# pnnl/FragNet

Measured on AMD Instinct MI355X. Metric: molecules/sec fwd+bwd (full training step), ESOL-shape batch=512 per GPU, higher is better.
Workload: dtype f32; 1 GPU; ESOL finetune batch=512 fp32 (BASELINE configs[1]): FragNetFineTune 4 layers x 4 heads, emb 128, FTHead3 128/1024/1024/512, drop 0.1; synthetic ESOL-shape molecules (synth.py); per_gpu_batch=512, global_batch=512, parallelism=dp1, overlap=off, graph_replays=736, eager_fallbacks=0, step=plan+zero_grad+fwd+mse+bwd+adam, atoms=13334, bond_graph_edges=200112

## Files before the change

### fragnet_amd/csrc/encoder.hip

```cpp
#include <hip/hip_runtime.h>
#include <algorithm>
#include <mutex>
#include <stdint.h>

#include "fn_internal.h"

namespace {
using fni::fail;
using fni::launch_status;
using fni::tune;
using fni::prof_event;
using fni::GatFwdArgs;
using fni::prep_gat_fwd;
using fni::launch_gat_fwd;
using fni::launch_gat_fwd_pair;
using fni::launch_gat_fwd_lin;
using fni::launch_gat_fwd_pair_lin;
using fni::GatBwdOneArgs;
using fni::CuTask;
using fni::CuTasks;
using fni::prep_gat_bwd_one;
using fni::launch_gat_bwd_one3;
using fni::launch_gat_cu;
using fni::launch_linear128_group;
// ... 7 lines not shown
#include "shared_bodies.inc"

constexpr int kRowDotsBwdBlocks = 512;

struct RowDotsBwdArgs {
    const float *g_s_sorted, *feat, *A;
    int lda, off, J;
    fn_gat_plan pl;
    float* g_feat;
    float* part;
    const float* addend;
    int g_is_orig, nblk;
    const float *cu_out2, *cu_sigma;
    float *cu_c, *cu_u;
    const int32_t* n_real;
};
__device__ __forceinline__ void row_dots_sorted_bwd_range(const RowDotsBwdArgs& T, float (*sR)[FN_D], int64_t e0, int64_t e1, int vb) {
    const float* __restrict__ g_s_sorted = T.g_s_sorted;
    const float* __restrict__ feat = T.feat;
    const float* __restrict__ A = T.A;
    const int lda = T.lda, off = T.off, J = T.J, g_is_orig = T.g_is_orig;
    const fn_gat_plan& pl = T.pl;
    float* g_feat = T.g_feat;
    float* __restrict__ part = T.part;
    const float* addend = T.addend;
    const int lane = threadIdx.x & 31, hw = threadIdx.x >> 5;
    float4 a[8], q[8];
#pragma unroll
    for (int i = 0; i < 8; ++i) {
        a[i] = (i < J) ? ld4(A + i * lda + off + lane * 4) : make_float4(0.f, 0.f, 0.f, 0.f);
// ... 45 lines not shown
                fma4(q[i], gs, v);
            }
        }
        if (addend) { const float4 a0 = ld4(addend + e * FN_D + lane * 4); acc.x += a0.x; acc.y += a0.y; acc.z += a0.z; acc.w += a0.w; }
        st4(g_feat + e * FN_D + lane * 4, acc);
    }
#pragma unroll
    for (int i = 0; i < 8; ++i) {
        if (i < J) {
            st4(&sR[hw][lane * 4], q[i]);
            __syncthreads();
            if (threadIdx.x < FN_D) {
                float v = 0.f;
#pragma unroll
                for (int w = 0; w < kRows; ++w) v += sR[w][threadIdx.x];
                part[(size_t)(i * FN_D + threadIdx.x) * FN_MAX_PART + vb] = v;
            }
            __syncthreads();
        }
    }
}
__device__ __forceinline__ void row_dots_sorted_bwd_body(const RowDotsBwdArgs& T, float (*sR)[FN_D], int vb, int nb) {
    const int64_t m_live = T.n_real && *T.n_real < T.pl.m_real ? (int64_t)*T.n_real : T.pl.m_real;
    const int64_t groups = (T.pl.m_real + kRows - 1) / kRows, per = (groups + nb - 1) / nb;
    const int64_t live_blocks = (m_live + per * kRows - 1) / (per * kRows);
    const int64_t g0 = (int64_t)xcd_block_real(vb, nb, (int)(live_blocks < nb ? live_blocks : nb)) * per, g1 = g0 + per < groups ? g0 + per : groups;
    const int64_t e1 = g1 * kRows < m_live ? g1 * kRows : m_live;
    row_dots_sorted_bwd_range(T, sR, g0 * kRows < e1 ? g0 * kRows : e1, e1, vb);
}
__global__ __launch_bounds__(kBlock) void k_row_dots_sorted_bwd(RowDotsBwdArgs T) {
    __shared__ float sR[kRows][FN_D];
// ... 322 lines not shown
    return o;
}

bool have_mol(const fn_encoder* e) {
    return e->n_mols > 0 && e->mol_atoms.rowptr && e->mol_frags.rowptr && e->mol_atoms.n_seg == e->n_mols && e->mol_frags.n_seg == e->n_mols;
}
bool pad_skip_on(const fn_encoder* e) {
    return tune(FN_TUNE_PAD_SKIP) != 0 && one_pass_on(e) && have_mol(e) && e->mol_contiguous != 0 && e->counts_dev != nullptr && e->variant == 0;
}
bool tail_mol_on(const fn_encoder* e) {
    return tune(FN_TUNE_MOL_TAIL) != 0 && e->mol_contiguous != 0 && have_mol(e) && e->variant == 0 &&
           (e->heads == 2 || e->heads == 4 || e->heads == 8) && e->F > 0 && e->EF > 0 && e->frag.m > 1 && e->n_mols <= FN_MAX_PART &&
           !((uintptr_t)e->ws & 15);
}

struct LevelScratch {
    float *g_h, *dz, *pz, *g_s_dst, *part_a, *part_e, *part_rd, *wg_ws;
    float* cdot;
};
struct BwdLayout {
    float* g_pre[kLevels + 1];
    float* g_frags;
    LevelScratch lv[FN_MAX_LAYERS][kLevels], frag;
    int64_t total;
};

BwdLayout bwd_layout(const fn_encoder* e, float* ws) {
    BwdLayout o{};
    Bump b(ws);
    const int H = e->heads;
// ... 118 lines not shown
    if (et.mode == 0) et.s_sorted = s_sorted;
    return et;
}
inline NodeScalarEpi node_scalars(const LevelView& v) { return NodeScalarEpi{v.att, v.s_dst, v.s_src, v.att_w, 0, v.src_off, v.H}; }
inline LinTask proj_task(const LevelView& v, int k_task = 0) {
    LinTask t{v.W, v.x, v.Wt, v.bias, v.a.h, v.rows, fn_act_epilogue{nullptr, 0.f, 0, 0, 0, nullptr}, node_scalars(v), 0, 0, k_task};
    t.n_real = v.n_real;
    return t;
}

struct ParamWork {
    int n_a = 0, n_e = 0;
    int n_rd = 0;
};
inline fni::AttParamGrads att_param_grads(const LevelView& v, const LevelWeights& g, const LevelScratch& sc, int n_a, int n_e) {
    return fni::AttParamGrads{v.H, sc.part_a, n_a, sc.part_e, n_e, v.et, v.att, v.att_w, v.src_off, g.att, g.embW, g.embb};
}
int edge_term_colsum(ParamGradQueue& rq, const LevelView& v, const LevelWeights& g, const LevelScratch& sc, int n_rd) {
    return rq.colsum(sc.part_rd, n_rd, v.H * FN_D, g.att, v.att_w, v.mid_off);
}
int level_params(ParamGradQueue& rq, const LevelView& v, const LevelWeights& g, const LevelScratch& sc, const ParamWork& o, hipStream_t launch_on) {
    FN_TRY(rq.finalize(att_param_grads(v, g, sc, o.n_a, o.n_e)));
    if (o.n_rd) FN_TRY(edge_term_colsum(rq, v, g, sc, o.n_rd));
    return rq.wgrad(fni::ProjWgrad{sc.g_h, v.x, v.K, v.rows, sc.wg_ws, v.n_real, g.W, g.bias}, launch_on);
}

int launch_gat_bwd_src(const GatBwdSrcArgs& A, int heads, hipStream_t st) {
    if (A.nblk == 0) return 0;
    FN_TRY(with_heads(heads, [&](auto H) { hipLaunchKernelGGL((k_gat_bwd_src<FN_CV(H), kBwdRows>), dim3(A.nblk), dim3(kBwdRows * 32), 0, st, A); }));
    return launch_status("fn_gat_bwd_src_f32");
}

int bwd_src_and_edge_term(const LevelView& v, const LevelScratch& sc, const float* g_out, float* g_h, const float* feat, float* g_feat,
                          bool accumulate, int* n_part_a, int* n_rd, hipStream_t st) {
    const int heads = v.H;
    GatBwdSrcArgs A;
    if (int rc = prep_gat_bwd_src(g_out, v.a.h, sc.pz, sc.g_s_dst, v.att, v.att_w, 0, v.src_off, v.pl, g_h, sc.part_a, n_part_a, heads, &A)) return rc;
    *n_rd = v.pl->m_real > 0 ? row_grid(v.pl->m_real, tune(FN_TUNE_RD_BLOCKS) > 0 ? tune(FN_TUNE_RD_BLOCKS) : kRowDotsBwdBlocks) : 0;
    if (*n_rd == 0) return launch_gat_bwd_src(A, heads, st);
    const RowDotsBwdArgs T{sc.dz, feat, v.att, v.att_w, v.mid_off, heads, *v.pl, g_feat, sc.part_rd, accumulate ? (const float*)g_feat : nullptr, 1, *n_rd};
    if (A.nblk == 0) {
        hipLaunchKernelGGL(k_row_dots_sorted_bwd, dim3(T.nblk), dim3(kBlock), 0, st, T);
        return launch_status("edge-term backward");
    }
    FN_TRY(with_heads(heads, [&](auto H) { hipLaunchKernelGGL((k_gat_bwd_src_rd<FN_CV(H), kBwdRows>), dim3(A.nblk + T.nblk), dim3(kBlock), 0, st, A, T); }));
    return launch_status("source pass + edge-term backward");
}

static int launch_lin_rd(LinTasks& T, const RowDotsBwdArgs& R, hipStream_t st) {
    int blocks = 0, live = 0;
    bool aligned = true;
    for (int i = 0; i < T.n; ++i) {
        if (T.t[i].M <= 0) continue;
        LinTask t = T.t[i];
        if (((uintptr_t)t.X | (uintptr_t)t.Bt | (uintptr_t)t.Y | (uintptr_t)t.bias | (uintptr_t)t.mk.y) & 15) aligned = false;
// ... 52 lines not shown
int launch_tail_bwd(const fn_encoder* e, const EncLayout& lay, const BwdLayout& bw, const EncOutputs& y, const EncOutputs& gy, bool accumulate_fbond,
                    int* n_part, hipStream_t st, bool one_pass_dots = false, bool* rider_done = nullptr) {
    const int H = e->heads, l = e->n_layers - 1;
    const LevelView vf = level_view(e, lay, l, LV_FRAG), va = level_view(e, lay, l, LV_ATOM), vfb = level_view(e, lay, l, LV_FBOND);
    const LevelScratch& sf = bw.frag;
    const float *y_atoms = y.y[LV_ATOM], *y_frags = y.y[LV_FRAG], *g_atoms = gy.y[LV_ATOM], *g_frags = gy.y[LV_FRAG];
    TailBwdArgs T{};
    T.ext = reinterpret_cast<const MolExt*>(lay.mol_ext);  T.n_mols = (int)e->n_mols;  T.counts_dev = e->counts_dev;
    T.g_atoms = g_atoms;  T.g_frags = g_frags;  T.g_pooled = e->g_pooled;  T.y_atoms = y_atoms;  T.y_frags = y_frags;  T.scale = gate_scale(e);
    T.g_pre_atoms = bw.g_pre[LV_ATOM];  T.g_pre_frags = bw.g_pre[LV_FRAG];  T.a2f_index = e->a2f.index;  T.n_atoms = e->N;  T.force_global = tune(FN_TUNE_MOL_TAIL) == 2;
    int n_e = 0, n_a = 0;
    FN_TRY(prep_gat_bwd_dst(bw.g_pre[LV_FRAG], vf.a.h, vf.a.p, &vf.et, vf.pl, 0.2f, nullptr, sf.dz, sf.pz, sf.g_s_dst, nullptr, &n_e, H, &T.D));
    FN_TRY(prep_gat_bwd_src(bw.g_pre[LV_FRAG], vf.a.h, sf.pz, sf.g_s_dst, vf.att, vf.att_w, 0, vf.src_off, vf.pl, bw.g_frags, sf.part_a, &n_a, H, &T.S));
    T.R = RowDotsBwdArgs{sf.dz, vfb.a.raw, vf.att, vf.att_w, vf.mid_off, H, *vf.pl, bw.g_pre[LV_FBOND], sf.part_rd,
                         accumulate_fbond ? (const float*)bw.g_pre[LV_FBOND] : (const float*)nullptr, 1, 0};
    if (one_pass_dots) {
        const LevelScratch &sa = bw.lv[l][LV_ATOM], &sfb = bw.lv[l][LV_FBOND];
        T.cu_out = va.a.raw;  T.cu_out2 = va.a.o2;  T.cu_sigma = va.a.sg;  T.cu_c = sa.cdot;  T.cu_u = sa.g_s_dst;
        if (H == 4) { T.R.cu_out2 = vfb.a.o2;  T.R.cu_sigma = vfb.a.sg;  T.R.cu_c = sfb.cdot;  T.R.cu_u = sfb.g_s_dst; }
    }
    if (((uintptr_t)y_atoms | (uintptr_t)y_frags | (uintptr_t)g_atoms | (uintptr_t)g_frags | (uintptr_t)e->g_pooled) & 15)
        return fail(FN_EINVAL, "fragment tail backward: gradients must be 16-byte aligned");
    AdamRide R{};
    if (rider_done) {
        *rider_done = false;
        if (tune(FN_TUNE_RIDER_AT) == 1 && e->adam_rider) {
            R = make_adam_ride(e->adam_rider, (int)e->n_mols, kBlock, tune(FN_TUNE_RIDER_PIECES));
            *rider_done = R.nblk > 0;
        }
    }
// ... 39 lines not shown
    int n_a = 0, n_e = 0;
    if (tail_mol) {
        int n_part = 0;
        bool rode = false;
        FN_TRY(launch_tail_bwd(e, lay, bw, y, gy, have_fbond, &n_part, hs, one_pass, one_pass ? &rode : nullptr));
        if (rode) rq.rider = nullptr;
        FN_TRY(rq.finalize(att_param_grads(vf, gf, sf, n_part, 0)));
        FN_TRY(edge_term_colsum(rq, vf, gf, sf, n_part));
        have_atoms = have_fbond = true;
        out->tail_dots_atoms = one_pass;  out->tail_dots_fbond = one_pass && H == 4;
    } else if (have_frags && lite) {
        g_frags_h = bw.g_pre[LV_FRAG];
        have_g_frags_h = true;
    } else if (have_frags && edge) {
        FN_TRY(fn_gat_bwd_dst_f32(bw.g_pre[LV_FRAG], vf.a.h, vf.a.p, &vf.et, vf.pl, 0.2f, nullptr, nullptr, sf.pz, sf.g_s_dst, sf.part_e, &n_e, H, hs));
        FN_TRY(fn_gat_bwd_src_f32(bw.g_pre[LV_FRAG], vf.a.h, sf.pz, sf.g_s_dst, vf.att, vf.att_w, 0, vf.src_off, vf.pl, bw.g_frags, sf.part_a, &n_a, H, hs));
        FN_TRY(rq.finalize(att_param_grads(vf, gf, sf, n_a, n_e)));
        have_g_frags_h = true;
    } else if (have_frags) {
        FN_TRY(fn_gat_bwd_dst_f32(bw.g_pre[LV_FRAG], vf.a.h, vf.a.p, &vf.et, vf.pl, 0.2f, nullptr, sf.dz, sf.pz, sf.g_s_dst, nullptr, &n_e, H, hs));
        int gr = 0;
        FN_TRY(bwd_src_and_edge_term(vf, sf, bw.g_pre[LV_FRAG], bw.g_frags, lay.L[l].lv[LV_FBOND].raw, bw.g_pre[LV_FBOND], have_fbond, &n_a, &gr, hs));
        if (gr) have_fbond = true;
        FN_TRY(rq.finalize(att_param_grads(vf, gf, sf, n_a, 0)));
        if (gr) FN_TRY(edge_term_colsum(rq, vf, gf, sf, gr));
        have_g_frags_h = true;
    }
    if (have_g_frags_h) {
        FN_TRY(launch_gather_rows4(g_frags_h, e->a2f.index, bw.g_pre[LV_ATOM], e->N, 32, have_atoms ? (const float*)bw.g_pre[LV_ATOM] : (const float*)nullptr, hs,
                                   "fn_encoder_backward: gather(a2f)"));
        have_atoms = true;
// ... 4 lines not shown

int encoder_backward_one(const fn_encoder* e, const EncLayout& lay, const BwdLayout& bw, const RngPlan& rng, const EncOutputs& y,
                         const EncOutputs& gy, const fn_layer_weights* grads, hipStream_t hs) {
    const int H = e->heads, NL = e->n_layers;
    const bool no_fb = e->variant != 0;
    ParamGradQueue rq;
    rq.st = hs;
    rq.defer_mixed = tune(FN_TUNE_GEMM_COLAUNCH) != 0;
    rq.rider = e->adam_rider;
    struct Parts { int n_a = 0, n_e = 0; };
    auto one_level = [&](const LevelView& v, const LevelScratch& sc, Parts* n, GatBwdOneArgs* A) -> int {
        FN_TRY(prep_gat_bwd_one(bw.g_pre[v.lv], v.a.h, v.a.p, sc.cdot, sc.g_s_dst, &v.et, v.att, v.att_w, 0, v.src_off, v.pl, 0.2f, sc.g_h, nullptr, sc.dz,
                                sc.part_a, &n->n_a, sc.part_e, &n->n_e, H, A));
        A->p_edge_major = 1;
        A->n_real = v.n_real;
        return 0;
    };
    auto scratch = [&](const LevelView& v) -> const LevelScratch& { return bw.lv[v.layer][v.lv]; };
    auto cu_add = [&](CuTasks& T, const LevelView& v) {
        const LevelScratch& sc = scratch(v);
        if (v.rows > 0) T.t[T.n++] = CuTask{bw.g_pre[v.lv], v.a.raw, v.a.o2, v.a.sg, 1.f, sc.cdot, sc.g_s_dst, v.rows, 0, 0};
    };
    auto cu_epi = [&](const LevelView& v, bool raw, bool dots = true) {
        const LevelScratch& sc = scratch(v);
        return CuEpi{raw ? v.a.raw : nullptr, v.a.o2, v.a.sg, dots ? sc.cdot : nullptr, sc.g_s_dst, H};
    };

    LastGrads top{};
    FN_TRY(last_layer_output_grads(e, lay, bw, y, gy, grads, rq, true, hs, &top));
    bool have_atoms = top.have[LV_ATOM], have_bond = top.have[LV_BOND], have_fbond = top.have[LV_FBOND] && !no_fb;
// ... 43 lines not shown
            product(vfb_up, vfb, nullptr, cu_epi(vfb, false));
            nxt_fbond = true;
        }
        RowDotsBwdArgs R{};
        if (have_atoms) {
            FN_TRY(level_params(rq, va, ga, sa, ParamWork{na.n_a, 0}, hs));
            if (l) {
                product(va, va_below, nullptr, cu_epi(va_below, false));
                nxt_atoms = true;
            }
            if (gr) {
                const bool have_b_now = pend_b || (last && have_bond);
                R = RowDotsBwdArgs{sa.dz, vb.a.raw, va.att, va.att_w, va.mid_off, H, *va.pl, rd_rows_ride ? nullptr : bw.g_pre[LV_BOND], sa.part_rd,
                                   (!rd_rows_ride && have_b_now) ? (const float*)bw.g_pre[LV_BOND] : nullptr, 1, gr};
                R.n_real = vb.n_real;
                FN_TRY(edge_term_colsum(rq, va, ga, sa, gr));
                if (!pend_b) {
                    const LevelScratch& sb = scratch(vb);
                    if (H == 4 && e->atom.m_real == e->E) { R.cu_out2 = vb.a.o2;  R.cu_sigma = vb.a.sg;  R.cu_c = sb.cdot;  R.cu_u = sb.g_s_dst; }
                    else cu_add(cu_after, vb);
                }
                nxt_bond = true;
            }
        }
        if (R.nblk && !rd_rows_ride && pend_b) {
            FN_TRY(launch_lin_rd(T, RowDotsBwdArgs{}, hs));
            T = LinTasks{};
        }
        FN_TRY(launch_lin_rd(T, R, hs));

// ... 337 lines not shown

        if (have[LV_ATOM]) {
            int n_a = 0, n_e = 0, gr = 0;
            FN_TRY(fn_gat_bwd_dst_f32(bw.g_pre[LV_ATOM], va.a.h, va.a.p, &va.et, va.pl, 0.2f, nullptr, sa.dz, sa.pz, sa.g_s_dst, nullptr, &n_e, H, st));
            FN_TRY(bwd_src_and_edge_term(va, sa, bw.g_pre[LV_ATOM], sa.g_h, vb.a.raw, bw.g_pre[LV_BOND], have[LV_BOND], &n_a, &gr, hs));
            if (gr) have[LV_BOND] = true;
            FN_TRY(level_params(rq, va, level_weights(g, LV_ATOM), sa, ParamWork{n_a, 0, gr}, hs));
            if (l) input_grad(va, sa);
        }

        Parts nb, nfb;
        auto dst_pass = [&](const LevelView& v, const LevelScratch& sc, Parts* n) {
            return fn_gat_bwd_dst_f32(bw.g_pre[v.lv], v.a.h, v.a.p, &v.et, v.pl, 0.2f, nullptr, nullptr, sc.pz, sc.g_s_dst, sc.part_e, &n->n_e, H, st);
        };
        auto src_pass = [&](const LevelView& v, const LevelScratch& sc, Parts* n) {
            return fn_gat_bwd_src_f32(bw.g_pre[v.lv], v.a.h, sc.pz, sc.g_s_dst, v.att, v.att_w, 0, v.src_off, v.pl, sc.g_h, sc.part_a, &n->n_a, H, st);
        };
        if (have[LV_BOND]) FN_TRY(dst_pass(vb, sb, &nb));
        if (have[LV_FBOND]) FN_TRY(dst_pass(vfb, sfb, &nfb));
        if (have[LV_BOND]) FN_TRY(src_pass(vb, sb, &nb));
        if (have[LV_FBOND]) FN_TRY(src_pass(vfb, sfb, &nfb));
        if (have[LV_FBOND]) {
            if (l) input_grad(vfb, sfb);
            FN_TRY(level_params(rq, vfb, level_weights(g, LV_FBOND), sfb, ParamWork{nfb.n_a, nfb.n_e}, hs));
        }
        if (have[LV_BOND]) {
            FN_TRY(level_params(rq, vb, level_weights(g, LV_BOND), sb, ParamWork{nb.n_a, nb.n_e}, hs));
            if (l) input_grad(vb, sb);
        }
        if (dxT.n) FN_TRY(launch_linear128_group(dxT, hs));
        for (Level v : kProjected) have[v] = nxt[v];
// ... 67 lines not shown
```

### fragnet_amd/csrc/fn_internal.h

```cpp
#pragma once
#include <hip/hip_runtime.h>
#include <stdint.h>
#include <type_traits>

#include "fragnet_hip.h"

#define FNI_HIDDEN __attribute__((visibility("hidden")))

namespace fni {
FNI_HIDDEN int fail(int code, const char* what);
FNI_HIDDEN int launch_status(const char* where);
FNI_HIDDEN int tune(int key);
FNI_HIDDEN unsigned long long* stamps(int64_t* n_u64);

struct MolExt {
    int a0, na;
    int b0, nb;
    int f0, nf;
    int c0, nc;
    int eb0, meb;
    int ea0, mea;
    int ef0, mef;
    int ec0, mec;
};
// ... 63 lines not shown
                                       const FwdMask* mkb = nullptr);
struct GatBwdOneArgs {
    const float *g_out, *h, *p_sorted, *cdot, *g_s_dst, *att;
    int att_w, dst_off, src_off;
    fn_edge_term et;
    fn_gat_plan pl;
    float slope;
    float *g_h, *part_a, *part_e, *dz_sorted, *g_s_orig;
    int rows_per_hw, nblk;
    int p_edge_major;
    const float* x_src;
    const int32_t* n_real;
    int tier6;
    float* dz_em;
    unsigned long long* stamps;
};
struct CuTask {
    const float *g, *out, *out2, *sigma;
    float scale;
    float *c, *u;
    int64_t n;
    int first, nblk;
};
constexpr int kMaxCuTasks = 4;
struct CuTasks { CuTask t[kMaxCuTasks]; int n; };
struct GsdSegTask {
    const float* dz;
    const int32_t* rowptr;
    int pos_base;
    int64_t n;
// ... 23 lines not shown
    const float* p;
    float* out;
    const int32_t* n_real;
};
FNI_HIDDEN int launch_attn_readout(const AttnReadoutTask* tasks, int n_tasks, int heads, hipStream_t st);
FNI_HIDDEN int launch_linear_dx(const fn_linear_dx_task* tasks, int n_tasks, hipStream_t st);
enum { RT_FINALIZE = 0, RT_COLSUM = 1, RT_WGRAD = 2 };
struct ReduceTask {
    int kind, first, nblk, H;
    const float *p0, *p1;
    int n0, n1;
    fn_edge_term et;
    const float* att;
    int att_w, dst_off, src_off, K;
    float *o0, *o1, *o2;
    int ld, off, cls, pad_;
};
constexpr int kMaxReduceTasks = 36;
struct ReduceTasks {
    ReduceTask t[kMaxReduceTasks];
    int first[kMaxReduceTasks + 1];
    int n;
};
struct WgradTask {
    const float *dY, *X;
    float* part;
    int64_t M;
    int rpb, first;
    int K;
    const int32_t* n_real;
};
constexpr int kMaxWgradTasks = 3 * FN_MAX_LAYERS;
struct WgradTasks {
    WgradTask t[kMaxWgradTasks];
    int n, K;
};
struct AttParamGrads {
    int H;
    const float* part_a;  int n_a;
    const float* part_e;  int n_e;
    fn_edge_term et;
    const float* att;  int att_w, src_off;
    float *g_att, *g_embW, *g_embb;
};
struct ProjWgrad {
    const float *g_h, *x;
    int K;
    int64_t M;
    float* ws;
    const int32_t* n_real;
    float *dW, *db;
};
struct FNI_HIDDEN ParamGradQueue {
    hipStream_t st = nullptr;
    bool defer_mixed = false;
    fn_adam_slice* rider = nullptr;
    int finalize(const AttParamGrads& a);
    int colsum(const float* part, int n_rows, int cols, float* out, int ld, int off);
    int wgrad(const ProjWgrad& p, hipStream_t launch_on);
    int flush(bool last = false);
private:
    ReduceTasks T{};
    WgradTasks W{}, W0{};
    int blocks = 0, wblocks = 0, w0blocks = 0;
    int w_reduce[kMaxWgradTasks] = {};
    int push(ReduceTask t, int nblk);
    void size_group128();
    int flush_wgrad();
};
FNI_HIDDEN int prof_event(int i, hipStream_t st);
FNI_HIDDEN bool bad_edge_term(const fn_edge_term* et, int64_t m);
}

// ... 87 lines not shown
__device__ __forceinline__ void fma4(float4& acc, float s, float4 v) {
    acc.x = fmaf(s, v.x, acc.x); acc.y = fmaf(s, v.y, acc.y);
    acc.z = fmaf(s, v.z, acc.z); acc.w = fmaf(s, v.w, acc.w);
}

__device__ __forceinline__ int xcd_block(int b, int nwg) {
    const int q = nwg >> 3, r = nwg & 7, x = b & 7;
    return (x < r ? x * (q + 1) : r * (q + 1) + (x - r) * q) + (b >> 3);
}
#ifndef FN_XCD_REAL
#define FN_XCD_REAL 1
#endif
#ifndef FN_PAD_BLOCK_EXIT
#define FN_PAD_BLOCK_EXIT 1
#endif
__device__ __forceinline__ int xcd_block_real(int b, int nwg, int nreal) {
    if (!FN_XCD_REAL || nreal >= nwg || nreal <= 0) return xcd_block(b, nwg);
    const int x = b & 7, k = b >> 3;
    const int qr = (nreal >> 3) + (x < (nreal & 7) ? 1 : 0);
    if (k < qr) return xcd_block(b, nreal);
    int before = 0;
#pragma unroll
    for (int y = 0; y < 7; ++y)
        if (y < x) before += ((nwg >> 3) + (y < (nwg & 7) ? 1 : 0)) - ((nreal >> 3) + (y < (nreal & 7) ? 1 : 0));
    return nreal + before + (k - qr);
}
__device__ __forceinline__ void block_groups(int64_t n_rows, int rb, int64_t& begin, int64_t& end) {
    const int64_t groups = (n_rows + rb - 1) / rb;
    const int64_t per = (groups + gridDim.x - 1) / gridDim.x;
    begin = (int64_t)xcd_block(blockIdx.x, gridDim.x) * per;
// ... 154 lines not shown
```

### fragnet_amd/csrc/gat_bwd_one.inc

```

using fni::GatBwdOneArgs;

template <int NX> struct OneRaw {
    int pos;
    i32x2u tp, dq;
    f32x2u x[NX ? NX : 1];
};

template <int H, int KL, int RB, bool DF = false, bool EN = false>
__device__ __forceinline__ void gat_bwd_one_rows(const GatBwdOneArgs& A, float (*sA)[2 * FN_D], float (*sP)[8][kWfLd], int blk0, int se,
                                                 int rows_per_hw, int bid) {
    const float* __restrict__ g_out = A.g_out;
    const float* __restrict__ h = A.h;
    const float* __restrict__ cdot = A.cdot;
    const float* __restrict__ g_s_dst = A.g_s_dst;
    const fn_edge_term& et = A.et;
    const fn_gat_plan& pl = A.pl;
    const float slope = A.slope;
    float* __restrict__ g_h = A.g_h;
    float* __restrict__ dz_sorted = A.dz_sorted;
    float* __restrict__ g_s_orig = A.g_s_orig;
    constexpr int LPH = 32 / H;
    constexpr int NE = KL ? KL : 1;
    constexpr int NG = (2 * LPH >= 12 && KL == 1) ? 12 : 8;
// ... 231 lines not shown
    stamp(14, false);
    st4(&sA[hw][lane * 4], qd);
    st4(&sA[hw][FN_D + lane * 4], qs);
    if (KL) {
#pragma unroll
        for (int k = 0; k <= NE; ++k) {
            const float v = head_sum<LPH>(pw[k]);
            if (j == 0) sP[hw][head][k == NE ? FN_MAX_EDGE_K : k] = v;
        }
    }
    __syncthreads();
    for (int c = threadIdx.x; c < 2 * FN_D; c += blockDim.x) {
        float a = 0.f;
#pragma unroll
        for (int w = 0; w < RB; ++w) a += sA[w][c];
        A.part_a[(size_t)c * FN_MAX_PART + bid] = a;
    }
    if (KL) {
        const int ne = H * (K + 1);
        for (int i = threadIdx.x; i < ne; i += blockDim.x) {
            const int hh = i / (K + 1), k = i % (K + 1);
            const int kk = (k == K) ? FN_MAX_EDGE_K : k;
            float a = 0.f;
#pragma unroll
            for (int w = 0; w < RB; ++w) a += sP[w][hh][kk];
            A.part_e[(size_t)bid * ne + i] = a;
        }
    }
    stamp(15, true);
}

template <int H, int KL, int RB, bool DF = false, bool EN = false>
__device__ __forceinline__ void gat_bwd_one_body(const GatBwdOneArgs& A, float (*sA)[2 * FN_D], float (*sP)[8][kWfLd], int bid, int nblk) {
    const int n = (int)A.pl.n, per = RB * A.rows_per_hw;
    const int nr = A.n_real ? *A.n_real : n;
    const int blk0 = xcd_block_real(bid, nblk, A.n_real ? (nr + per - 1) / per : nblk) * per;
    if (FN_PAD_BLOCK_EXIT && blk0 >= nr && !A.stamps) {
        const int lane = threadIdx.x & 31, hw = threadIdx.x >> 5, end = blk0 + per < n ? blk0 + per : n;
        for (int s = blk0 + hw; s < end; s += RB) st4(A.g_h + (size_t)s * FN_D + lane * 4, make_float4(0.f, 0.f, 0.f, 0.f));
        for (int c = threadIdx.x; c < 2 * FN_D; c += blockDim.x) A.part_a[(size_t)c * FN_MAX_PART + bid] = 0.f;
        if (KL) {
            const int ne = H * (A.et.K + 1);
            for (int i = threadIdx.x; i < ne; i += blockDim.x) A.part_e[(size_t)bid * ne + i] = 0.f;
        }
        return;
    }
    gat_bwd_one_rows<H, KL, RB, DF, EN>(A, sA, sP, blk0, blk0 + per < n ? blk0 + per : n, A.rows_per_hw, bid);
}
template <int H, int KL, int RB, bool DF = false, bool EN = false>
__global__ __launch_bounds__(RB * 32, 3) void k_gat_bwd_one(GatBwdOneArgs A) {
    __shared__ float sA[RB][2 * FN_D];
    __shared__ float sP[RB][8][kWfLd];
    gat_bwd_one_body<H, KL, RB, DF, EN>(A, sA, sP, (int)blockIdx.x, (int)gridDim.x);
}
template <int H, int RB, bool EN = false>
// ... 77 lines not shown
```

### fragnet_amd/csrc/gat_bwd_two.inc

```

template <int NE> struct BwdRaw {
    int pos;
    i32x2u sp, sq, eq;
    f32x2u pp;
    f32x2u x[NE];
};

struct GatBwdDstArgs {
    const float *g_out, *h, *p_sorted;
    fn_edge_term et;
    fn_gat_plan pl;
    float slope;
    float *dz_sorted, *g_s_orig, *pz_src, *g_s_dst, *part_e;
    int rows_per_hw, nblk;
};
template <int H, int KL, int RB>
__device__ __forceinline__ void gat_bwd_dst_rows(const GatBwdDstArgs& A, float (*sP)[8][kWfLd], int blk0, int te, int rows_per_hw, int bid) {
    const float* __restrict__ g_out = A.g_out;
    const float* __restrict__ h = A.h;
    const float* __restrict__ p_sorted = A.p_sorted;
    const fn_edge_term& et = A.et;
    const fn_gat_plan& pl = A.pl;
    const float slope = A.slope;
    float* __restrict__ dz_sorted = A.dz_sorted;
// ... 186 lines not shown
    const int blk0 = xcd_block(bid, nblk) * RB * A.rows_per_hw, n = (int)A.pl.n;
    gat_bwd_dst_rows<H, KL, RB>(A, sP, blk0, blk0 + RB * A.rows_per_hw < n ? blk0 + RB * A.rows_per_hw : n, A.rows_per_hw, bid);
}
template <int H, int KL, int RB>
__global__ __launch_bounds__(RB * 32) void k_gat_bwd_dst(GatBwdDstArgs A) {
    __shared__ float sP[RB][8][kWfLd];
    gat_bwd_dst_body<H, KL, RB>(A, sP, (int)blockIdx.x, (int)gridDim.x);
}

struct GatBwdSrcArgs {
    const float *g_out, *h, *pz_src, *g_s_dst, *att;
    int att_w, dst_off, src_off;
    fn_gat_plan pl;
    float *g_h, *part_a;
    int rows_per_hw, nblk;
};
template <int H, int RB>
__device__ __forceinline__ void gat_bwd_src_rows(const GatBwdSrcArgs& A, float (*sA)[2 * FN_D], int blk0, int se, int rows_per_hw, int bid) {
    const float* __restrict__ g_out = A.g_out;
    const float* __restrict__ h = A.h;
    const float* __restrict__ pz_src = A.pz_src;
    const float* __restrict__ g_s_dst = A.g_s_dst;
    const float* __restrict__ att = A.att;
    const int att_w = A.att_w, dst_off = A.dst_off, src_off = A.src_off;
    const fn_gat_plan& pl = A.pl;
    float* __restrict__ g_h = A.g_h;
    float* __restrict__ part_a = A.part_a;
    constexpr int LPH = 32 / H;
    const int lane = threadIdx.x & 31, head = lane / LPH, j = lane % LPH, hw = threadIdx.x >> 5;
    const int m = (int)pl.m, n = (int)pl.n;
// ... 91 lines not shown
        if (cur_deg >= 0) {
            fma4(acc, cur_gsd, ad);
            fma4(acc, gss, as);
            st4(g_h + (size_t)s * FN_D + lane * 4, acc);
            fma4(qd, cur_gsd, hr);
            fma4(qs, gss, hr);
        }
    }
    st4(&sA[hw][lane * 4], qd);
    st4(&sA[hw][FN_D + lane * 4], qs);
    __syncthreads();
    for (int c = threadIdx.x; c < 2 * FN_D; c += blockDim.x) {
        float a = 0.f;
#pragma unroll
        for (int w = 0; w < RB; ++w) a += sA[w][c];
        part_a[(size_t)c * FN_MAX_PART + bid] = a;
    }
}

template <int H, int RB>
__device__ __forceinline__ void gat_bwd_src_body(const GatBwdSrcArgs& A, float (*sA)[2 * FN_D], int bid, int nblk) {
    const int blk0 = xcd_block(bid, nblk) * RB * A.rows_per_hw, n = (int)A.pl.n;
    gat_bwd_src_rows<H, RB>(A, sA, blk0, blk0 + RB * A.rows_per_hw < n ? blk0 + RB * A.rows_per_hw : n, A.rows_per_hw, bid);
}
template <int H, int RB>
__global__ __launch_bounds__(RB * 32) void k_gat_bwd_src(GatBwdSrcArgs A) {
    __shared__ float sA[RB][2 * FN_D];
    gat_bwd_src_body<H, RB>(A, sA, (int)blockIdx.x, (int)gridDim.x);
}


// ... 57 lines not shown
```

### fragnet_amd/csrc/mol_tail.inc

```

struct TailFwdArgs {
    const MolExt* ext;  int n_mols;  const int32_t* counts_dev;
    const float* atoms_new;  const int32_t* a2f_rowptr;  const int32_t* a2f_perm;  int32_t a2f_base, a2f_items;
    float* frags;
    const float* att;  int att_w, dst_off, src_off, mid_off;
    float *s_dst, *s_src;
    const float* feat;  float* s_sorted;
    GatFwdArgs G;
    const float* y_atoms;  float* pooled;
    int force_global;
};

constexpr int kTailNF = 32, kTailME = 128;
template <int H> constexpr int tail_bwd_nf() { return H == 8 ? 32 : 24; }

template <int H>
struct TailFwdLds {
    float F[kTailNF][FN_D];
    float S[kRows][2 * FN_D];
    float sd[kTailNF][H], ss[kTailNF][H];
    float e[H][kTailME];
    int rp[kTailNF + 1];
    int src[kTailME];
};
// ... 371 lines not shown
        }
        st4(T.R.g_feat + (size_t)(x.c0 + el) * FN_D + lane * 4, acc);
        if (T.R.cu_c)
            row_cu_dots<H>(acc, v, (el == hw || !T.R.cu_out2) ? cv0 : ld4(T.R.cu_out2 + (size_t)(x.c0 + el) * FN_D + lane * 4),
                           (el == hw || !T.R.cu_out2) ? cs0 : T.R.cu_sigma[(size_t)(x.c0 + el) * H + lane / (32 / H)], T.R.cu_c, T.R.cu_u, x.c0 + el, lane);
    }
    __syncthreads();
    float* const P = L.FG;
    st4(P + hw * 2 * FN_D + lane * 4, qd);
    st4(P + hw * 2 * FN_D + FN_D + lane * 4, qs);
    __syncthreads();
    {
        float v = 0.f;
#pragma unroll
        for (int w = 0; w < kRows; ++w) v += P[w * 2 * FN_D + tid];
        T.S.part_a[(size_t)tid * FN_MAX_PART + mol] = v;
    }
    __syncthreads();
#pragma unroll
    for (int h = 0; h < H; ++h) st4(P + (hw * H + h) * FN_D + lane * 4, q[h]);
    __syncthreads();
    for (int c = tid; c < H * FN_D; c += kBlock) {
        float v = 0.f;
#pragma unroll
        for (int w = 0; w < kRows; ++w) v += P[w * H * FN_D + c];
        T.R.part[(size_t)c * FN_MAX_PART + mol] = v;
    }
    for (int i0 = hw; i0 < x.na; i0 += 4 * kRows) {
        int fr[4];
        float4 yv[4], ga[4], ov[4], o2v[4];
        float sg[4];
#pragma unroll
        for (int u = 0; u < 4; ++u) {
            if (i0 == hw) { fr[u] = fr0[u];  yv[u] = yv0[u];  ga[u] = ga0[u];  ov[u] = ov0[u];  o2v[u] = o2v0[u];  sg[u] = sg0[u];  continue; }
            if (T.cu_c) {
                const size_t ia = (size_t)(x.a0 + (i0 + u * kRows < x.na ? i0 + u * kRows : i0));
                ov[u] = ld4(T.cu_out + ia * FN_D + lane * 4);  o2v[u] = T.cu_out2 ? ld4(T.cu_out2 + ia * FN_D + lane * 4) : zero;
                sg[u] = T.cu_out2 ? T.cu_sigma[ia * H + lane / (32 / H)] : 0.f;
            } else { ov[u] = zero;  o2v[u] = zero;  sg[u] = 0.f; }
            const int i = x.a0 + (i0 + u * kRows < x.na ? i0 + u * kRows : i0);
            fr[u] = (int)T.a2f_index[i] - x.f0;
// ... 55 lines not shown
    static_assert(kBwdRows == kRows && kBwdRows * 32 == kBlock, "the cores run 8 half-waves per block");
    constexpr int kTailNF = tail_bwd_nf<H>();
    static_assert(sizeof(TailBwdLds<H>) <= 64 * 1024 && 2 * kTailNF >= kRows * H && 2 * kTailNF * FN_D >= kRows * 2 * FN_D, "LDS tile");
    __shared__ TailBwdLds<H> L;
    if (R.nblk && (int)blockIdx.x >= R.first) { adam_ride(R);  return; }
    const int mol = (int)blockIdx.x, lane = threadIdx.x & 31, hw = threadIdx.x >> 5;
    const MolExt x = T.ext[mol];
    const int n_real = T.counts_dev ? *T.counts_dev : T.n_mols;
    if (mol >= n_real) {
        const float4 zero = make_float4(0.f, 0.f, 0.f, 0.f);
        for (int i = x.a0 + hw; i < x.a0 + x.na; i += kRows) st4(T.g_pre_atoms + (size_t)i * FN_D + lane * 4, zero);
        if (T.R.g_feat && !T.R.addend)
            for (int c = x.c0 + hw; c < x.c0 + x.nc; c += kRows) st4(T.R.g_feat + (size_t)c * FN_D + lane * 4, zero);
        if (T.cu_c) for (int i = x.a0 * H + (int)threadIdx.x; i < (x.a0 + x.na) * H; i += kBlock) { T.cu_c[i] = 0.f;  if (T.cu_u) T.cu_u[i] = 0.f; }
        if (T.R.cu_c) for (int c = x.c0 * H + (int)threadIdx.x; c < (x.c0 + x.nc) * H; c += kBlock) { T.R.cu_c[c] = 0.f;  if (T.R.cu_u) T.R.cu_u[c] = 0.f; }
        T.S.part_a[(size_t)threadIdx.x * FN_MAX_PART + mol] = 0.f;
        for (int c = threadIdx.x; c < H * FN_D; c += kBlock) T.R.part[(size_t)c * FN_MAX_PART + mol] = 0.f;
        return;
    }
    if (x.nf <= kTailNF && x.mec <= kTailME && x.nc <= kTailME && T.force_global == 0) tail_bwd_lds<H>(T, x, mol, L);
    else tail_bwd_global<H>(T, x, mol, reinterpret_cast<float(*)[2 * FN_D]>(L.FG));
}
```

### fragnet_amd/csrc/param_grads.hip

```cpp
#include <hip/hip_runtime.h>
#include <algorithm>
#include <stdint.h>

#include "fn_internal.h"

namespace {
using fni::fail;
using fni::launch_status;
using fni::tune;
using fni::ReduceTask;
using fni::ReduceTasks;
using fni::WgradTask;
using fni::WgradTasks;
using fni::kMaxReduceTasks;
using fni::kMaxWgradTasks;
using fni::RT_FINALIZE;
using fni::RT_COLSUM;
using fni::RT_WGRAD;

#include "zero2.inc"
#include "shared_bodies.inc"
#include "linear128.inc"

constexpr int kWgChunk = 32;
// ... 171 lines not shown

template <int CTW, int NH>
__global__ __launch_bounds__(1024) void k_wgrad_reduce(const float* __restrict__ part, int n_rows, int K,
                                                       float* __restrict__ dW, float* __restrict__ db) {
    __shared__ float sm[32 * 33];
    wgrad_reduce_body<CTW, NH>(blockIdx.x, sm, part, n_rows, K, dW, db);
}

__device__ __forceinline__ float colmajor_sum_32(const float* __restrict__ col, int n_rows) {
    const int lane = threadIdx.x & 31;
    float v = 0.f, v1 = 0.f, v2 = 0.f, v3 = 0.f;
    int r = lane;
    for (; r + 96 < n_rows; r += 128) { v += col[r];  v1 += col[r + 32];  v2 += col[r + 64];  v3 += col[r + 96]; }
    for (; r < n_rows; r += 32) v += col[r];
    v = (v + v1) + (v2 + v3);
#pragma unroll
    for (int off = 16; off > 0; off >>= 1) v += __shfl_xor(v, off);
    return v;
}
template <int CTW, int NH, bool PLAIN = false>
__device__ __forceinline__ void wgrad_reduce_strip(int vb, float* sm, const float* __restrict__ part, int n_rows, int K,
                                                   float* __restrict__ dW, float* __restrict__ db) {
    constexpr int XW = 16 * CTW * NH;
    constexpr int PW = 128 * XW + 128;
    const int c4 = threadIdx.x & 255, rg = threadIdx.x >> 8;
    const int col0 = vb * 1024 + c4 * 4;
    float4 acc = make_float4(0.f, 0.f, 0.f, 0.f);
    if (col0 < PW) {
        float4 a1 = acc, a2 = acc, a3 = acc;
        int r = rg;
// ... 108 lines not shown
                                                       float* __restrict__ g_embW, float* __restrict__ g_embb, int H) {
    __shared__ float sm[1200];
    gat_finalize_body(blockIdx.x, sm, part_a, n_a, part_e, n_e, et, att, att_w, dst_off, src_off, g_att, g_embW, g_embb, H);
}

__global__ __launch_bounds__(1024) void k_reduce_tasks(ReduceTasks T, AdamRide R) {
    __shared__ float sm[16 * 256];
    if (R.nblk && (int)blockIdx.x >= R.first) { adam_ride(R);  return; }
    int ti = 0;
    while (ti + 1 < T.n && (int)blockIdx.x >= T.first[ti + 1]) ++ti;
    const ReduceTask& t = T.t[ti];
    const int vb = (int)blockIdx.x - T.first[ti];
    if (t.kind == RT_FINALIZE) {
        if (vb < 2 * FN_D / 32) {
            const int col = vb * 32 + (threadIdx.x >> 5);
            const float v = colmajor_sum_32(t.p0 + (size_t)col * FN_MAX_PART, t.n0);
            if ((threadIdx.x & 31) == 0) {
                const int DH = FN_D / t.H, cc = col & 127, part = col >> 7;
                t.o0[(cc / DH) * t.att_w + (part ? t.src_off : t.dst_off) + (cc % DH)] = v;
            }
        } else {
            gat_finalize_body(2 * FN_D, sm, t.p0, t.n0, t.p1, t.n1, t.et, t.att, t.att_w, t.dst_off, t.src_off, t.o0, t.o1, t.o2, t.H);
        }
    } else if (t.kind == RT_COLSUM) {
        const int col = vb * 32 + (threadIdx.x >> 5);
        const float v = colmajor_sum_32(t.p0 + (size_t)col * FN_MAX_PART, t.n0);
        if ((threadIdx.x & 31) == 0) t.o0[(col / FN_D) * t.ld + t.off + (col % FN_D)] = v;
    } else {
        switch (t.cls) {
            case 0: wgrad_reduce_strip<1, 1>(vb, sm, t.p0, t.n0, t.K, t.o0, t.o1); break;
            case 1: wgrad_reduce_strip<1, 2>(vb, sm, t.p0, t.n0, t.K, t.o0, t.o1); break;
            case 2: wgrad_reduce_strip<4, 2>(vb, sm, t.p0, t.n0, t.K, t.o0, t.o1); break;
            case 4: wgrad_reduce_strip<4, 2, true>(vb, sm, t.p0, t.n0, t.K, t.o0, t.o1); break;
            default: wgrad_reduce_strip<6, 2>(vb, sm, t.p0, t.n0, t.K, t.o0, t.o1); break;
        }
    }
}

constexpr int kWgCtw[5] = {1, 1, 4, 6, 4}, kWgNh[5] = {1, 2, 2, 2, 2};
constexpr int kWgClassDirect128 = 4;
inline int wgrad_class(int K, bool mixed = false) { return K <= 16 ? (mixed ? 1 : 0) : K <= 32 ? 1 : K <= 128 ? 2 : K <= 192 ? 3 : -1; }
// ... 46 lines not shown
    if (rc == 0 && R.nblk > 0) rider->launched = 1;
    return rc;
}
int ParamGradQueue::push(ReduceTask t, int nblk) {
    if (T.n == kMaxReduceTasks) { if (int rc = flush()) return rc; }
    t.first = blocks;  t.nblk = nblk;
    T.first[T.n] = blocks;
    T.t[T.n++] = t;
    blocks += nblk;
    return 0;
}
int ParamGradQueue::finalize(const AttParamGrads& a) {
    ReduceTask t{};
    t.kind = RT_FINALIZE;  t.H = a.H;  t.p0 = a.part_a;  t.n0 = a.n_a;  t.p1 = a.part_e;  t.n1 = a.n_e;  t.et = a.et;
    t.att = a.att;  t.att_w = a.att_w;  t.dst_off = 0;  t.src_off = a.src_off;  t.o0 = a.g_att;  t.o1 = a.g_embW;  t.o2 = a.g_embb;
    return push(t, 2 * FN_D / 32 + (a.et.mode == 2 ? 1 : 0));
}
int ParamGradQueue::colsum(const float* part, int n_rows, int cols, float* out, int ld, int off) {
    ReduceTask t{};
    t.kind = RT_COLSUM;  t.p0 = part;  t.n0 = n_rows;  t.o0 = out;  t.ld = ld;  t.off = off;
    if (cols % 32) return fail(FN_EINVAL, "deferred column sum: column count must be a multiple of 32");
    return push(t, cols / 32);
}
int ParamGradQueue::wgrad(const ProjWgrad& p, hipStream_t launch_on) {
    const int K = p.K;
    const int64_t M = p.M;
    float* ws = p.ws;
    if (M == 0) {
        hipLaunchKernelGGL(k_zero2_i32, dim3(flat_grid(128 * (K + 1), kGridCap)), dim3(kBlock), 0, launch_on,
                           reinterpret_cast<int32_t*>(p.dW), (int64_t)128 * K, reinterpret_cast<int32_t*>(p.db), (int64_t)128);
        return launch_status("weight gradient (empty)");
    }
    ReduceTask t{};
    int grid = 0;
    if (K == FN_D) {
// ... 108 lines not shown
```

Before: 706,300 molecules/s.

## Store attention/edge-term partial sums row-major for coalesced writes

Switches the per-block partial-sum buffers (part_a, part_rd) from column-major (column stride FN_MAX_PART) to row-major with a leading dimension, so each block writes its partial row contiguously instead of with strided scatters. The reduction kernels get a new row-major column-sum path that reads rows coalesced by 32 columns and transposes through shared memory before a shuffle reduction. This trades scattered producer writes for an extra LDS transpose and a __syncthreads in the reducer. It is on by default via FN_PART_ROWMAJOR.

```diff
diff --git a/fragnet_amd/csrc/encoder.hip b/fragnet_amd/csrc/encoder.hip
--- a/fragnet_amd/csrc/encoder.hip
+++ b/fragnet_amd/csrc/encoder.hip
@@ -45,6 +45,7 @@
     const float *cu_out2, *cu_sigma;
     float *cu_c, *cu_u;
     const int32_t* n_real;
+    int part_ld;
 };
 __device__ __forceinline__ void row_dots_sorted_bwd_range(const RowDotsBwdArgs& T, float (*sR)[FN_D], int64_t e0, int64_t e1, int vb) {
     const float* __restrict__ g_s_sorted = T.g_s_sorted;
@@ -120,7 +121,7 @@
                 float v = 0.f;
 #pragma unroll
                 for (int w = 0; w < kRows; ++w) v += sR[w][threadIdx.x];
-                part[(size_t)(i * FN_D + threadIdx.x) * FN_MAX_PART + vb] = v;
+                part[part_at(T.part_ld, vb, i * FN_D + (int)threadIdx.x)] = v;
             }
             __syncthreads();
         }
@@ -473,6 +474,8 @@
            !((uintptr_t)e->ws & 15);
 }
 
+constexpr int part_a_ld() { return FN_PART_ROWMAJOR ? 2 * FN_D : 0; }
+constexpr int part_rd_ld(int H) { return FN_PART_ROWMAJOR ? H * FN_D : 0; }
 struct LevelScratch {
     float *g_h, *dz, *pz, *g_s_dst, *part_a, *part_e, *part_rd, *wg_ws;
     float* cdot;
@@ -621,10 +624,10 @@
     int n_rd = 0;
 };
 inline fni::AttParamGrads att_param_grads(const LevelView& v, const LevelWeights& g, const LevelScratch& sc, int n_a, int n_e) {
-    return fni::AttParamGrads{v.H, sc.part_a, n_a, sc.part_e, n_e, v.et, v.att, v.att_w, v.src_off, g.att, g.embW, g.embb};
+    return fni::AttParamGrads{v.H, sc.part_a, n_a, sc.part_e, n_e, v.et, v.att, v.att_w, v.src_off, g.att, g.embW, g.embb, part_a_ld()};
 }
 int edge_term_colsum(ParamGradQueue& rq, const LevelView& v, const LevelWeights& g, const LevelScratch& sc, int n_rd) {
-    return rq.colsum(sc.part_rd, n_rd, v.H * FN_D, g.att, v.att_w, v.mid_off);
+    return rq.colsum(sc.part_rd, n_rd, v.H * FN_D, g.att, v.att_w, v.mid_off, part_rd_ld(v.H));
 }
 int level_params(ParamGradQueue& rq, const LevelView& v, const LevelWeights& g, const LevelScratch& sc, const ParamWork& o, hipStream_t launch_on) {
     FN_TRY(rq.finalize(att_param_grads(v, g, sc, o.n_a, o.n_e)));
@@ -636,6 +639,13 @@
     if (A.nblk == 0) return 0;
     FN_TRY(with_heads(heads, [&](auto H) { hipLaunchKernelGGL((k_gat_bwd_src<FN_CV(H), kBwdRows>), dim3(A.nblk), dim3(kBwdRows * 32), 0, st, A); }));
     return launch_status("fn_gat_bwd_src_f32");
+}
+
+int engine_bwd_src(const LevelView& v, const LevelScratch& sc, const float* g_out, float* g_h, int* n_part_a, hipStream_t st) {
+    GatBwdSrcArgs A;
+    if (int rc = prep_gat_bwd_src(g_out, v.a.h, sc.pz, sc.g_s_dst, v.att, v.att_w, 0, v.src_off, v.pl, g_h, sc.part_a, n_part_a, v.H, &A)) return rc;
+    A.part_ld = part_a_ld();
+    return launch_gat_bwd_src(A, v.H, st);
 }
 
 int bwd_src_and_edge_term(const LevelView& v, const LevelScratch& sc, const float* g_out, float* g_h, const float* feat, float* g_feat,
@@ -643,9 +653,11 @@
     const int heads = v.H;
     GatBwdSrcArgs A;
     if (int rc = prep_gat_bwd_src(g_out, v.a.h, sc.pz, sc.g_s_dst, v.att, v.att_w, 0, v.src_off, v.pl, g_h, sc.part_a, n_part_a, heads, &A)) return rc;
+    A.part_ld = part_a_ld();
     *n_rd = v.pl->m_real > 0 ? row_grid(v.pl->m_real, tune(FN_TUNE_RD_BLOCKS) > 0 ? tune(FN_TUNE_RD_BLOCKS) : kRowDotsBwdBlocks) : 0;
     if (*n_rd == 0) return launch_gat_bwd_src(A, heads, st);
-    const RowDotsBwdArgs T{sc.dz, feat, v.att, v.att_w, v.mid_off, heads, *v.pl, g_feat, sc.part_rd, accumulate ? (const float*)g_feat : nullptr, 1, *n_rd};
+    RowDotsBwdArgs T{sc.dz, feat, v.att, v.att_w, v.mid_off, heads, *v.pl, g_feat, sc.part_rd, accumulate ? (const float*)g_feat : nullptr, 1, *n_rd};
+    T.part_ld = part_rd_ld(heads);
     if (A.nblk == 0) {
         hipLaunchKernelGGL(k_row_dots_sorted_bwd, dim3(T.nblk), dim3(kBlock), 0, st, T);
         return launch_status("edge-term backward");
@@ -728,6 +740,7 @@
     FN_TRY(prep_gat_bwd_src(bw.g_pre[LV_FRAG], vf.a.h, sf.pz, sf.g_s_dst, vf.att, vf.att_w, 0, vf.src_off, vf.pl, bw.g_frags, sf.part_a, &n_a, H, &T.S));
     T.R = RowDotsBwdArgs{sf.dz, vfb.a.raw, vf.att, vf.att_w, vf.mid_off, H, *vf.pl, bw.g_pre[LV_FBOND], sf.part_rd,
                          accumulate_fbond ? (const float*)bw.g_pre[LV_FBOND] : (const float*)nullptr, 1, 0};
+    T.S.part_ld = part_a_ld();  T.R.part_ld = part_rd_ld(H);
     if (one_pass_dots) {
         const LevelScratch &sa = bw.lv[l][LV_ATOM], &sfb = bw.lv[l][LV_FBOND];
         T.cu_out = va.a.raw;  T.cu_out2 = va.a.o2;  T.cu_sigma = va.a.sg;  T.cu_c = sa.cdot;  T.cu_u = sa.g_s_dst;
@@ -797,7 +810,7 @@
         have_g_frags_h = true;
     } else if (have_frags && edge) {
         FN_TRY(fn_gat_bwd_dst_f32(bw.g_pre[LV_FRAG], vf.a.h, vf.a.p, &vf.et, vf.pl, 0.2f, nullptr, nullptr, sf.pz, sf.g_s_dst, sf.part_e, &n_e, H, hs));
-        FN_TRY(fn_gat_bwd_src_f32(bw.g_pre[LV_FRAG], vf.a.h, sf.pz, sf.g_s_dst, vf.att, vf.att_w, 0, vf.src_off, vf.pl, bw.g_frags, sf.part_a, &n_a, H, hs));
+        FN_TRY(engine_bwd_src(vf, sf, bw.g_pre[LV_FRAG], bw.g_frags, &n_a, hs));
         FN_TRY(rq.finalize(att_param_grads(vf, gf, sf, n_a, n_e)));
         have_g_frags_h = true;
     } else if (have_frags) {
@@ -832,6 +845,7 @@
                                 sc.part_a, &n->n_a, sc.part_e, &n->n_e, H, A));
         A->p_edge_major = 1;
         A->n_real = v.n_real;
+        A->part_ld = part_a_ld();
         return 0;
     };
     auto scratch = [&](const LevelView& v) -> const LevelScratch& { return bw.lv[v.layer][v.lv]; };
@@ -905,6 +919,7 @@
                 R = RowDotsBwdArgs{sa.dz, vb.a.raw, va.att, va.att_w, va.mid_off, H, *va.pl, rd_rows_ride ? nullptr : bw.g_pre[LV_BOND], sa.part_rd,
                                    (!rd_rows_ride && have_b_now) ? (const float*)bw.g_pre[LV_BOND] : nullptr, 1, gr};
                 R.n_real = vb.n_real;
+                R.part_ld = part_rd_ld(H);
                 FN_TRY(edge_term_colsum(rq, va, ga, sa, gr));
                 if (!pend_b) {
                     const LevelScratch& sb = scratch(vb);
@@ -1272,7 +1287,7 @@
             return fn_gat_bwd_dst_f32(bw.g_pre[v.lv], v.a.h, v.a.p, &v.et, v.pl, 0.2f, nullptr, nullptr, sc.pz, sc.g_s_dst, sc.part_e, &n->n_e, H, st);
         };
         auto src_pass = [&](const LevelView& v, const LevelScratch& sc, Parts* n) {
-            return fn_gat_bwd_src_f32(bw.g_pre[v.lv], v.a.h, sc.pz, sc.g_s_dst, v.att, v.att_w, 0, v.src_off, v.pl, sc.g_h, sc.part_a, &n->n_a, H, st);
+            return engine_bwd_src(v, sc, bw.g_pre[v.lv], sc.g_h, &n->n_a, S(st));
         };
         if (have[LV_BOND]) FN_TRY(dst_pass(vb, sb, &nb));
         if (have[LV_FBOND]) FN_TRY(dst_pass(vfb, sfb, &nfb));
diff --git a/fragnet_amd/csrc/fn_internal.h b/fragnet_amd/csrc/fn_internal.h
--- a/fragnet_amd/csrc/fn_internal.h
+++ b/fragnet_amd/csrc/fn_internal.h
@@ -101,6 +101,7 @@
     int tier6;
     float* dz_em;
     unsigned long long* stamps;
+    int part_ld;
 };
 struct CuTask {
     const float *g, *out, *out2, *sigma;
@@ -154,7 +155,7 @@
     const float* att;
     int att_w, dst_off, src_off, K;
     float *o0, *o1, *o2;
-    int ld, off, cls, pad_;
+    int ld, off, cls, pld;
 };
 constexpr int kMaxReduceTasks = 36;
 struct ReduceTasks {
@@ -182,6 +183,7 @@
     fn_edge_term et;
     const float* att;  int att_w, src_off;
     float *g_att, *g_embW, *g_embb;
+    int part_ld;
 };
 struct ProjWgrad {
     const float *g_h, *x;
@@ -196,7 +198,7 @@
     bool defer_mixed = false;
     fn_adam_slice* rider = nullptr;
     int finalize(const AttParamGrads& a);
-    int colsum(const float* part, int n_rows, int cols, float* out, int ld, int off);
+    int colsum(const float* part, int n_rows, int cols, float* out, int ld, int off, int part_ld = 0);
     int wgrad(const ProjWgrad& p, hipStream_t launch_on);
     int flush(bool last = false);
 private:
@@ -314,6 +316,12 @@
 #ifndef FN_PAD_BLOCK_EXIT
 #define FN_PAD_BLOCK_EXIT 1
 #endif
+#ifndef FN_PART_ROWMAJOR
+#define FN_PART_ROWMAJOR 1
+#endif
+__device__ __forceinline__ size_t part_at(int ld, int row, int col) {
+    return ld ? (size_t)row * ld + col : (size_t)col * FN_MAX_PART + row;
+}
 __device__ __forceinline__ int xcd_block_real(int b, int nwg, int nreal) {
     if (!FN_XCD_REAL || nreal >= nwg || nreal <= 0) return xcd_block(b, nwg);
     const int x = b & 7, k = b >> 3;
diff --git a/fragnet_amd/csrc/gat_bwd_one.inc b/fragnet_amd/csrc/gat_bwd_one.inc
--- a/fragnet_amd/csrc/gat_bwd_one.inc
+++ b/fragnet_amd/csrc/gat_bwd_one.inc
@@ -269,7 +269,7 @@
         float a = 0.f;
 #pragma unroll
         for (int w = 0; w < RB; ++w) a += sA[w][c];
-        A.part_a[(size_t)c * FN_MAX_PART + bid] = a;
+        A.part_a[part_at(A.part_ld, bid, c)] = a;
     }
     if (KL) {
         const int ne = H * (K + 1);
@@ -293,7 +293,7 @@
     if (FN_PAD_BLOCK_EXIT && blk0 >= nr && !A.stamps) {
         const int lane = threadIdx.x & 31, hw = threadIdx.x >> 5, end = blk0 + per < n ? blk0 + per : n;
         for (int s = blk0 + hw; s < end; s += RB) st4(A.g_h + (size_t)s * FN_D + lane * 4, make_float4(0.f, 0.f, 0.f, 0.f));
-        for (int c = threadIdx.x; c < 2 * FN_D; c += blockDim.x) A.part_a[(size_t)c * FN_MAX_PART + bid] = 0.f;
+        for (int c = threadIdx.x; c < 2 * FN_D; c += blockDim.x) A.part_a[part_at(A.part_ld, bid, c)] = 0.f;
         if (KL) {
             const int ne = H * (A.et.K + 1);
             for (int i = threadIdx.x; i < ne; i += blockDim.x) A.part_e[(size_t)bid * ne + i] = 0.f;
diff --git a/fragnet_amd/csrc/gat_bwd_two.inc b/fragnet_amd/csrc/gat_bwd_two.inc
--- a/fragnet_amd/csrc/gat_bwd_two.inc
+++ b/fragnet_amd/csrc/gat_bwd_two.inc
@@ -224,6 +224,7 @@
     fn_gat_plan pl;
     float *g_h, *part_a;
     int rows_per_hw, nblk;
+    int part_ld;
 };
 template <int H, int RB>
 __device__ __forceinline__ void gat_bwd_src_rows(const GatBwdSrcArgs& A, float (*sA)[2 * FN_D], int blk0, int se, int rows_per_hw, int bid) {
@@ -345,7 +346,7 @@
         float a = 0.f;
 #pragma unroll
         for (int w = 0; w < RB; ++w) a += sA[w][c];
-        part_a[(size_t)c * FN_MAX_PART + bid] = a;
+        part_a[part_at(A.part_ld, bid, c)] = a;
     }
 }
 
diff --git a/fragnet_amd/csrc/mol_tail.inc b/fragnet_amd/csrc/mol_tail.inc
--- a/fragnet_amd/csrc/mol_tail.inc
+++ b/fragnet_amd/csrc/mol_tail.inc
@@ -409,7 +409,7 @@
         float v = 0.f;
 #pragma unroll
         for (int w = 0; w < kRows; ++w) v += P[w * 2 * FN_D + tid];
-        T.S.part_a[(size_t)tid * FN_MAX_PART + mol] = v;
+        T.S.part_a[part_at(T.S.part_ld, mol, tid)] = v;
     }
     __syncthreads();
 #pragma unroll
@@ -419,7 +419,7 @@
         float v = 0.f;
 #pragma unroll
         for (int w = 0; w < kRows; ++w) v += P[w * H * FN_D + c];
-        T.R.part[(size_t)c * FN_MAX_PART + mol] = v;
+        T.R.part[part_at(T.R.part_ld, mol, c)] = v;
     }
     for (int i0 = hw; i0 < x.na; i0 += 4 * kRows) {
         int fr[4];
@@ -505,8 +505,8 @@
             for (int c = x.c0 + hw; c < x.c0 + x.nc; c += kRows) st4(T.R.g_feat + (size_t)c * FN_D + lane * 4, zero);
         if (T.cu_c) for (int i = x.a0 * H + (int)threadIdx.x; i < (x.a0 + x.na) * H; i += kBlock) { T.cu_c[i] = 0.f;  if (T.cu_u) T.cu_u[i] = 0.f; }
         if (T.R.cu_c) for (int c = x.c0 * H + (int)threadIdx.x; c < (x.c0 + x.nc) * H; c += kBlock) { T.R.cu_c[c] = 0.f;  if (T.R.cu_u) T.R.cu_u[c] = 0.f; }
-        T.S.part_a[(size_t)threadIdx.x * FN_MAX_PART + mol] = 0.f;
-        for (int c = threadIdx.x; c < H * FN_D; c += kBlock) T.R.part[(size_t)c * FN_MAX_PART + mol] = 0.f;
+        T.S.part_a[part_at(T.S.part_ld, mol, (int)threadIdx.x)] = 0.f;
+        for (int c = threadIdx.x; c < H * FN_D; c += kBlock) T.R.part[part_at(T.R.part_ld, mol, c)] = 0.f;
         return;
     }
     if (x.nf <= kTailNF && x.mec <= kTailME && x.nc <= kTailME && T.force_global == 0) tail_bwd_lds<H>(T, x, mol, L);
diff --git a/fragnet_amd/csrc/param_grads.hip b/fragnet_amd/csrc/param_grads.hip
--- a/fragnet_amd/csrc/param_grads.hip
+++ b/fragnet_amd/csrc/param_grads.hip
@@ -209,6 +209,23 @@
     for (; r + 96 < n_rows; r += 128) { v += col[r];  v1 += col[r + 32];  v2 += col[r + 64];  v3 += col[r + 96]; }
     for (; r < n_rows; r += 32) v += col[r];
     v = (v + v1) + (v2 + v3);
+#pragma unroll
+    for (int off = 16; off > 0; off >>= 1) v += __shfl_xor(v, off);
+    return v;
+}
+__device__ __forceinline__ float rowmajor_sum_32(const float* __restrict__ part, int ld, int col0, int n_rows, float* sm) {
+    const int c = threadIdx.x & 31, lane = threadIdx.x >> 5;
+    const float* __restrict__ p = part + col0 + c;
+    float v = 0.f, v1 = 0.f, v2 = 0.f, v3 = 0.f;
+    int r = lane;
+    for (; r + 96 < n_rows; r += 128) {
+        v += p[(size_t)r * ld];  v1 += p[(size_t)(r + 32) * ld];  v2 += p[(size_t)(r + 64) * ld];  v3 += p[(size_t)(r + 96) * ld];
+    }
+    for (; r < n_rows; r += 32) v += p[(size_t)r * ld];
+    v = (v + v1) + (v2 + v3);
+    sm[lane * 33 + c] = v;
+    __syncthreads();
+    v = sm[(threadIdx.x & 31) * 33 + (threadIdx.x >> 5)];
 #pragma unroll
     for (int off = 16; off > 0; off >>= 1) v += __shfl_xor(v, off);
     return v;
@@ -347,7 +364,7 @@
     if (t.kind == RT_FINALIZE) {
         if (vb < 2 * FN_D / 32) {
             const int col = vb * 32 + (threadIdx.x >> 5);
-            const float v = colmajor_sum_32(t.p0 + (size_t)col * FN_MAX_PART, t.n0);
+            const float v = t.pld ? rowmajor_sum_32(t.p0, t.pld, vb * 32, t.n0, sm) : colmajor_sum_32(t.p0 + (size_t)col * FN_MAX_PART, t.n0);
             if ((threadIdx.x & 31) == 0) {
                 const int DH = FN_D / t.H, cc = col & 127, part = col >> 7;
                 t.o0[(cc / DH) * t.att_w + (part ? t.src_off : t.dst_off) + (cc % DH)] = v;
@@ -357,7 +374,7 @@
         }
     } else if (t.kind == RT_COLSUM) {
         const int col = vb * 32 + (threadIdx.x >> 5);
-        const float v = colmajor_sum_32(t.p0 + (size_t)col * FN_MAX_PART, t.n0);
+        const float v = t.pld ? rowmajor_sum_32(t.p0, t.pld, vb * 32, t.n0, sm) : colmajor_sum_32(t.p0 + (size_t)col * FN_MAX_PART, t.n0);
         if ((threadIdx.x & 31) == 0) t.o0[(col / FN_D) * t.ld + t.off + (col % FN_D)] = v;
     } else {
         switch (t.cls) {
@@ -434,11 +451,12 @@
     ReduceTask t{};
     t.kind = RT_FINALIZE;  t.H = a.H;  t.p0 = a.part_a;  t.n0 = a.n_a;  t.p1 = a.part_e;  t.n1 = a.n_e;  t.et = a.et;
     t.att = a.att;  t.att_w = a.att_w;  t.dst_off = 0;  t.src_off = a.src_off;  t.o0 = a.g_att;  t.o1 = a.g_embW;  t.o2 = a.g_embb;
+    t.pld = a.part_ld;
     return push(t, 2 * FN_D / 32 + (a.et.mode == 2 ? 1 : 0));
 }
-int ParamGradQueue::colsum(const float* part, int n_rows, int cols, float* out, int ld, int off) {
+int ParamGradQueue::colsum(const float* part, int n_rows, int cols, float* out, int ld, int off, int part_ld) {
     ReduceTask t{};
-    t.kind = RT_COLSUM;  t.p0 = part;  t.n0 = n_rows;  t.o0 = out;  t.ld = ld;  t.off = off;
+    t.kind = RT_COLSUM;  t.p0 = part;  t.n0 = n_rows;  t.o0 = out;  t.ld = ld;  t.off = off;  t.pld = part_ld;
     if (cols % 32) return fail(FN_EINVAL, "deferred column sum: column count must be a multiple of 32");
     return push(t, cols / 32);
 }
```

Measured after the change: 725,900 molecules/s (median of 6 runs). +2.8%, better.
